# marja-w/gan-des-midi-music-gen

Measured on AMD Instinct MI355X. Metric: GAN training samples/sec (G+D step), higher is better.
Workload: dtype bf16; 1 GPU; SIMNN G/D iteration, synthetic 128x256 spectrogram windows; per_gpu_batch=256, global_batch=256, mode=faithful, parallelism=dp1

## Files before the change

gan_des_midi_music_gen_amd/_lib.py:

```python
import ctypes
import os
import threading

_PKG = os.path.dirname(os.path.abspath(__file__))
_TAG = os.environ.get("GDM_LIB_TAG", "")
LIB_PATH = os.path.join(_PKG, "libgdm_hip" + (f"_{_TAG}" if _TAG else "") + ".so")

F32, BF16 = 0, 1
ACT_NONE, ACT_RELU, ACT_LEAKY, ACT_SIGMOID = 0, 1, 2, 3

_c = ctypes
_P, _I, _L, _F, _Z = _c.c_void_p, _c.c_int, _c.c_int64, _c.c_float, _c.c_size_t

class LinearBnJob(_c.Structure):
    _fields_ = [(n, _P) for n in ("x", "w", "bias", "gamma", "beta", "running_mean", "running_var",
                                  "num_batches_tracked", "y_out", "out", "save_mean", "save_invstd")] + \
               [(n, _I) for n in ("M", "N", "K", "groups", "stat_repeats")]


class DcnnAdam(_c.Structure):
    _fields_ = [("param", _P * 6), ("exp_avg", _P * 6), ("exp_avg_sq", _P * 6), ("hyper", _P), ("done", _P)]


class ConcatJob(_c.Structure):
    _fields_ = [("a", _P), ("b", _P), ("out", _P), ("M", _I), ("Ka", _I), ("Kb", _I)]


SIGNATURES = {
    "gdm_last_error": (_c.c_char_p, []),
    "gdm_version": (_I, []),
    "gdm_arch": (_c.c_char_p, []),
    "gdm_build_flavor": (_I, []),
    "gdm_gemm": (_I, [_P, _I, _L, _L, _P, _I, _L, _L, _P, _I, _L, _L, _I, _I, _I, _P, _P, _I, _F, _I, _I, _P, _Z, _P]),
    "gdm_bce_with_logits": (_I, [_P, _F, _I, _F, _P, _P, _I, _I, _P]),
    "gdm_adam_step": (_I, [_P, _P, _P, _P, _L, _I, _F, _F, _F, _F, _F, _P]),
    "gdm_adam_step_dev": (_I, [_P, _P, _P, _P, _L, _P, _P]),
    "gdm_adam_step_dev_pc": (_I, [_P, _P, _P, _P, _I, _I, _I, _P, _I, _P, _I, _P]),
    "gdm_stft_frames": (_I, [_P, _I, _L, _L, _I, _I, _I, _P, _P]),
    "gdm_power_spectrum": (_I, [_P, _L, _I, _I, _P, _P]),
    "gdm_power_to_db": (_I, [_P, _I, _I, _I, _F, _F, _P, _P]),
    "gdm_bn_workspace_bytes": (_Z, [_I, _I]),
    "gdm_bn_act_fwd": (_I, [_P, _I, _I, _P, _P, _P, _P, _P, _F, _F, _I, _P, _I, _P, _P, _I, _P, _Z, _P]),
    "gdm_bn_act_bwd": (_I, [_P, _P, _I, _P, _I, _I, _P, _P, _P, _I, _P, _P, _P, _P, _Z, _P]),
    "gdm_bn_stats": (_I, [_P, _I, _I, _P, _P, _P, _F, _F, _P, _P, _P, _Z, _P]),
    "gdm_bn_partial_chunks": (_I, [_I]),
    "gdm_bn_partials": (_I, [_P, _I, _I, _P, _P]),
    "gdm_bn_apply": (_I, [_P, _I, _I, _P, _P, _P, _P, _I, _P, _I, _P]),
    "gdm_bn_finalize": (_I, [_P, _I, _I, _I, _F, _F, _P, _P, _P, _P, _P, _P]),
    "gdm_simnn_gen_pack_bytes": (_Z, []),
    "gdm_simnn_gen_pack": (_I, [_P, _I, _P, _P, _P, _P]),
    "gdm_simnn_gen_first": (_I, [_P, _I, _I, _P, _P, _F, _F, _P, _P, _P, _P, _P, _P]),
    "gdm_simnn_gen_convt_chunks": (_I, [_I, _I]),
    "gdm_simnn_gen_convt_bn": (_I, [_I, _P, _P, _P, _P, _P, _I, _P, _P, _P, _P]),
    "gdm_simnn_gen_last": (_I, [_P, _P, _P, _P, _P, _P, _I, _P, _P]),
    "gdm_bias_act_fwd": (_I, [_P, _P, _I, _I, _I, _F, _P, _I, _P]),
    "gdm_act_bwd": (_I, [_P, _P, _I, _L, _I, _F, _P, _P]),
    "gdm_colsum": (_I, [_P, _I, _I, _I, _P, _P, _Z, _P]),
    "gdm_cast": (_I, [_P, _I, _P, _I, _L, _P]),
    "gdm_nonfinite_count": (_I, [_P, _I, _L, _P, _P]),
    "gdm_simnn_conv1_fwd": (_I, [_P, _P, _P, _I, _I, _I, _P, _P, _I, _P]),
    "gdm_simnn_conv1_fwd_pair": (_I, [_P, _P, _I, _P, _P, _I, _I, _I, _P, _P, _I, _P]),
    "gdm_simnn_conv2_pack_bytes": (_Z, [_I]),
    "gdm_simnn_conv2_pack": (_I, [_P, _I, _P, _P]),
    "gdm_simnn_conv2_fwd": (_I, [_P, _P, _P, _I, _I, _I, _P, _P, _I, _P]),
    "gdm_simnn_conv2_bwd_fused_workspace_bytes": (_Z, [_I, _I, _I]),
    "gdm_simnn_conv2_bwd_fused": (_I, [_P, _P, _P, _I, _I, _I, _P, _P, _P, _I, _I, _I, _P, _I, _P, _Z, _P]),
    "gdm_simnn_conv2_bwd_fused_finish": (_I, [_I, _I, _I, _P, _P, _P, _Z, _P]),
    "gdm_simnn_conv2_bwd_data": (_I, [_P, _P, _P, _I, _I, _I, _P, _I, _P]),
    "gdm_simnn_conv2_bwd_weight_workspace_bytes": (_Z, [_I, _I, _I]),
    "gdm_simnn_conv2_bwd_weight": (_I, [_P, _P, _P, _I, _I, _I, _P, _P, _I, _P, _Z, _P]),
    "gdm_simnn_conv1_bwd_weight_workspace_bytes": (_Z, [_I, _I, _I]),
    "gdm_simnn_conv1_bwd_weight": (_I, [_P, _P, _P, _I, _I, _I, _P, _P, _I, _I, _P, _Z, _P]),
    "gdm_simnn_conv1_bwd_data": (_I, [_P, _P, _P, _I, _I, _I, _P, _I, _P]),
    "gdm_simnn_adam_step": (_I, [_P, _P, _P, _P, _I, _I, _I, _P, _P, _P, _P, _P, _I, _P, _P, _I, _P, _P, _P]),
    "gdm_simnn_head_workspace_bytes": (_Z, [_I]),
    "gdm_simnn_head": (_I, [_P, _P, _P, _I, _I, _F, _F, _P, _P, _I, _P, _I, _P, _P, _P, _P, _Z, _P]),
    "gdm_linear_bn_act_max_rows": (_I, []),
    "gdm_linear_bn_act_fwd_multi": (_I, [_P, _I, _F, _F, _I, _I, _P]),
    "gdm_concat_cols_multi": (_I, [_P, _I, _P]),
    "gdm_linear_bn_act_fwd": (_I, [_P, _P, _P, _P, _P, _P, _P, _P, _F, _F, _I, _I, _I, _I, _I, _P, _P, _P, _P, _I, _I,
                                   _P]),
    "gdm_dcnn_fused_supported": (_I, [_I]),
    "gdm_dcnn_pack_bytes": (_Z, [_I]),
    "gdm_dcnn_pack": (_I, [_P, _P, _P, _P, _P, _P, _I, _P, _P]),
    "gdm_dcnn_fused_workspace_bytes": (_Z, [_I, _I, _I]),
    "gdm_dcnn_fused": (_I, [_P, _I, _P, _P, _I, _I, _F, _F, _P, _P, _P, _I, _I, _P, _P, _P, _P, _P, _P, _P, _Z, _P]),
# ... 44 lines not shown
```

gan_des_midi_music_gen_amd/functional.py:

```python
import contextlib

import torch

from . import ops
from .ops import ACT_LEAKY, ACT_NONE, ACT_RELU, ACT_SIGMOID, BF16, F32

_DEFAULT = {"dtype": F32}
_NAMES = {"fp32": F32, "f32": F32, "float32": F32, "bf16": BF16, "bfloat16": BF16, F32: F32, BF16: BF16}


def set_compute_dtype(name):
    _DEFAULT["dtype"] = _NAMES[name]


def get_compute_dtype():
    return _DEFAULT["dtype"]


@contextlib.contextmanager
def compute_dtype(name):
    old = _DEFAULT["dtype"]
    _DEFAULT["dtype"] = _NAMES[name]
    try:
        yield
    finally:
        _DEFAULT["dtype"] = old


def _f32c(t):
    return t.detach().contiguous() if t.dtype == torch.float32 else t.detach().float().contiguous()


def simnn_disc_prepare(w2, wf1, dt, out=None):
    n, k = wf1.shape
    if out is not None:
        pack, wf1p = out
        ops.simnn_conv2_pack(w2, dt, out=pack)
        ops.permute_pc(wf1, n, 32, k // 32, out=wf1p)
        return pack, wf1p
    pack = ops.simnn_conv2_pack(w2, dt)
    wf1p = ops.permute_pc(wf1, n, 32, k // 32, out_dtype=dt).view(n, k)
    return pack, wf1p


def simnn_disc_features(x, w1, b1, pack, b2, wf1p, bf1, dt, trunk_out=None):
    if trunk_out is None:
        x = _f32c(x)
        p1, code1 = ops.simnn_conv1_fwd(x, w1, b1, dt)
    else:
        p1, code1 = trunk_out
    p2, code2 = ops.simnn_conv2_fwd(p1, pack, b2)
    b = p1.shape[0]
    flat = p2.view(b, -1)
    if flat.shape[1] != wf1p.shape[1]:
        raise ValueError(f"Discriminator.fc1 expects {wf1p.shape[1]} features but this input gives {flat.shape[1]} "
                         "(construct Discriminator(input_hw=...) for this geometry)")
    h1 = ops.gemm(flat, wf1p.t(), bias_n=bf1, act=ACT_RELU, compute=dt)
    return h1, (x, p1, code1, flat, code2, h1)


def simnn_disc_forward(x, w1, b1, pack, b2, wf1p, bf1, wf2, bf2, dt, trunk_out=None):
    h1, saved = simnn_disc_features(x, w1, b1, pack, b2, wf1p, bf1, dt, trunk_out)
    p = ops.gemm(h1, wf2.t(), bias_n=bf2, act=ACT_SIGMOID, compute=dt)
    return p, saved + (p,)


def simnn_disc_backward_from_dh1(saved, dh1, pack, wf1p, dt, out=None, x_pair=None, w1_for_dx=None):
    x, p1, code1, flat, code2 = saved[:5]
    b = p1.shape[0]
    o = out if out is not None else [None] * 8
    n, k = wf1p.shape
    dwf1p = ops.gemm(dh1.t(), flat, compute=dt)
    dwf1 = ops.permute_pc(dwf1p, n, k // 32, 32, out=o[4]).view(n, k)
    dflat = ops.gemm(dh1, wf1p, compute=dt, out_dtype=dt)
    h1s, w1s = p1.shape[1], p1.shape[2]
    dp2 = dflat.view(b, h1s // 2, w1s // 2, 32)
    dw2, db2 = ops.simnn_conv2_bwd_weight(dp2, code2, p1, out=None if out is None else (o[2], o[3]))
    x0, x1 = x_pair if x_pair is not None else (x, None)
    dw1, db1, dp1 = ops.simnn_conv2_bwd_fused(dp2, code2, pack, code1, x0, x1,
                                              out=None if out is None else (o[0], o[1]), want_dp1=w1_for_dx is not None)
    dx = None
    if w1_for_dx is not None:
        dx = ops.simnn_conv1_bwd_data(dp1, code1, w1_for_dx.contiguous(), x0.shape[1], x0.shape[2])
    return dw1, db1, dw2, db2, dwf1, dx


def simnn_disc_backward(saved, dz, pack, wf1p, wf2, dt, out=None, x_pair=None, w1_for_dx=None):
    h1 = saved[5]
    b = h1.shape[0]
    o = out if out is not None else [None] * 8
    dz = dz.reshape(b, 1).contiguous()
    dwf2 = ops.gemm(dz.t(), h1, compute=dt, out=o[6])
    dbf2 = ops.colsum(dz, out=o[7])
    dh1 = ops.act_bwd(ops.gemm(dz, wf2, compute=dt), h1, act=ACT_RELU)
    dbf1 = ops.colsum(dh1, out=o[5])
    dw1, db1, dw2, db2, dwf1, dx = simnn_disc_backward_from_dh1(saved, dh1, pack, wf1p, dt, out, x_pair, w1_for_dx)
    return dw1, db1, dw2, db2, dwf1, dbf1, dwf2, dbf2, dx


def _anomaly_guard(cls):
    fwd, bwd = cls.forward, cls.backward

    def _tensors(xs):
        out = []
        for x in xs:
            if isinstance(x, torch.Tensor) and x.is_floating_point() and x.is_cuda:
                out.append(x.detach())
            elif isinstance(x, (tuple, list)):
                out.extend(_tensors(x))
        return out

    def forward(ctx, *args):
        if not torch.is_anomaly_enabled():
            return fwd(ctx, *args)
        ops.assert_finite(_tensors(args), f"Function '{cls.__name__}' received")
        out = fwd(ctx, *args)
        ops.assert_finite(_tensors(out if isinstance(out, (tuple, list)) else (out,)), f"Function '{cls.__name__}' returned")
        return out

    def backward(ctx, *grads):
        out = bwd(ctx, *grads)
        if torch.is_anomaly_enabled():
            ops.assert_finite(_tensors(grads), f"Function '{cls.__name__}Backward' received")
            ops.assert_finite(_tensors(out if isinstance(out, (tuple, list)) else (out,)),
                              f"Function '{cls.__name__}Backward' returned nan values:")
        return out

# ... 430 lines not shown
```

gan_des_midi_music_gen_amd/ops.py:

```python
import contextlib
import ctypes
import threading

import torch

from . import _lib
from ._lib import ACT_LEAKY, ACT_NONE, ACT_RELU, ACT_SIGMOID, BF16, F32, GdmError, check

_TORCH_DT = {F32: torch.float32, BF16: torch.bfloat16}


def torch_dtype(dt):
    return _TORCH_DT[dt]


def gdm_dtype(t):
    if t.dtype == torch.float32:
        return F32
    if t.dtype == torch.bfloat16:
        return BF16
    raise GdmError(f"unsupported tensor dtype {t.dtype} (fp32 or bf16 only)")


def _need_gpu(*ts):
# ... 49 lines not shown
def workspace_namespace(ns):
    prev = getattr(_ws_ns, "ns", None)
    _ws_ns.ns = ns
    try:
        yield
    finally:
        _ws_ns.ns = prev


def workspace(nbytes, device):
    key = (device.index, torch.cuda.current_stream(device).cuda_stream, getattr(_ws_ns, "ns", None))
    capturing = torch.cuda.is_current_stream_capturing()
    buf = _ws_cache.get(key)
    if buf is None or buf.numel() < nbytes:
        if buf is not None and (capturing or key in _ws_pinned):
            _ws_retired.append(buf)
        buf = torch.empty(max(int(nbytes), 1 << 20), dtype=torch.uint8, device=device)
        _ws_cache[key] = buf
    if capturing:
        _ws_pinned.add(key)
    return buf


def default_split_k(m, n, k, compute):
    tile, kt = (128, 32) if compute == BF16 else (64, 32)
    tiles = ((m + tile - 1) // tile) * ((n + tile - 1) // tile)
    ktiles = (k + kt - 1) // kt
    if tiles >= 128 or ktiles < 32:
        return 1
    target = 256 if compute == BF16 else 768
    return max(1, min(ktiles // 8, (target + tiles - 1) // tiles))


def gemm(a, b, *, bias_n=None, bias_m=None, act=ACT_NONE, slope=0.0, out_dtype=None, compute=F32, split_k=None,
         out=None):
    _need_gpu(a, b, bias_n, bias_m, out)
    assert a.dim() == 2 and b.dim() == 2 and a.shape[1] == b.shape[0], (a.shape, b.shape)
    m, k = a.shape
    n = b.shape[1]
    if out is None:
        out = torch.empty((m, n), dtype=_TORCH_DT[F32 if out_dtype is None else out_dtype], device=a.device)
    assert out.shape == (m, n)
    if split_k is None:
        split_k = default_split_k(m, n, k, compute)
    ws, ws_bytes = None, 0
    if split_k > 1:
        ws_bytes = split_k * m * n * 4
        ws = workspace(ws_bytes, a.device)
    lib = _lib.load()
    _call("gdm_gemm", _p(a), gdm_dtype(a), a.stride(0), a.stride(1), _p(b), gdm_dtype(b), b.stride(0), b.stride(1),
                       _p(out), gdm_dtype(out), out.stride(0), out.stride(1), m, n, k, _p(bias_n), _p(bias_m), act,
                       float(slope), compute, split_k, _p(ws), ws_bytes, _stream())
    return out


def bce_with_logits(x, target, *, grad_scale=1.0, want_grad=True, fuse_sigmoid_backward=False, loss_out=None,
                    accumulate_loss=False, dx_out=None):
    _need_gpu(x, loss_out, dx_out)
    x = x.reshape(-1)
    assert x.dtype == torch.float32 and x.is_contiguous()
    loss = loss_out if loss_out is not None else torch.empty(1, dtype=torch.float32, device=x.device)
    dx = dx_out if dx_out is not None else (torch.empty_like(x) if want_grad else None)
    if dx is not None:
        assert dx.is_contiguous() and dx.numel() == x.numel() and dx.dtype == torch.float32
    _call("gdm_bce_with_logits", _p(x), float(target), x.numel(), float(grad_scale), _p(loss), _p(dx),
                                           1 if fuse_sigmoid_backward else 0, 1 if accumulate_loss else 0, _stream())
    return loss, dx


def adam_step(p, g, m, v, step, lr, beta1, beta2, eps, grad_scale=1.0):
    _need_gpu(p, g, m, v)
    for t in (p, g, m, v):
        assert t.dtype == torch.float32 and t.is_contiguous() and t.numel() == p.numel()
    _call("gdm_adam_step", _p(p), _p(g), _p(m), _p(v), p.numel(), int(step), float(lr), float(beta1),
                                    float(beta2), float(eps), float(grad_scale), _stream())


def adam_hyper(device, lr, beta1, beta2, eps, grad_scale=1.0, step=0):
    h = torch.zeros(8, dtype=torch.float32)
    h[1], h[2], h[3], h[4], h[5] = lr, beta1, beta2, eps, grad_scale
    h.view(torch.int32)[0] = int(step)
    return h.to(device)


def adam_step_dev(p, g, m, v, hyper):
    _need_gpu(p, g, m, v, hyper)
    assert hyper.numel() == 8 and hyper.dtype == torch.float32
    _call("gdm_adam_step_dev", _p(p), _p(g), _p(m), _p(v), p.numel(), _p(hyper), _stream())


def adam_step_dev_pc(p, g_pc, m, v, n, c, pix, shadow_pc, hyper, advance_step=False):
    _need_gpu(p, g_pc, m, v, shadow_pc, hyper)
    for t in (p, g_pc, m, v):
        assert t.dtype == torch.float32 and t.is_contiguous() and t.numel() == n * c * pix, (t.shape, n, c, pix)
    assert shadow_pc.is_contiguous() and shadow_pc.numel() == n * c * pix
    _call("gdm_adam_step_dev_pc", _p(p), _p(g_pc), _p(m), _p(v), n, c, pix, _p(shadow_pc), gdm_dtype(shadow_pc),
          _p(hyper), 1 if advance_step else 0, _stream())


SIMNN_ADAM_RECORD_INTS = 1056


def simnn_adam_step(p_big, g_big_pc, m_big, v_big, n, c, pix, shadow_pc, p_small, g_small, m_small, v_small, conv2_weight,
                    pack, hyper, done):
    _need_gpu(p_big, g_big_pc, m_big, v_big, shadow_pc, p_small, g_small, m_small, v_small, conv2_weight, pack, hyper, done)
    for t in (p_big, g_big_pc, m_big, v_big):
# ... 609 lines not shown
```

gan_des_midi_music_gen_amd/train.py:

```python
import torch

from . import dp
from . import functional as Fn
from . import ops


class FlatBuffers:

    ALIGN = 64

    def __init__(self, params, extra=0, local=0):
        params = [p for p in params]
        assert params, "no parameters"
        dev = params[0].device
        self.params = params
        self.numel = sum(p.numel() for p in params)
        big = max(range(len(params)), key=lambda i: params[i].numel())
        order = [i for i in range(len(params)) if i != big] + [big]
        n_small = self.numel - params[big].numel()
        assert extra % 4 == 0 and 0 <= local <= extra
        self.n_small = (n_small + self.ALIGN - 1) // self.ALIGN * self.ALIGN
        self.n_pad = self.n_small - n_small
        self.n_extra = extra
        self.n_local = local
# ... 177 lines not shown
            torch.cuda.current_stream().wait_event(self._gen_event)
        return self._last_generated

    def invalidate_weights(self):
        self._prepared = None

    def _refresh_operands(self):
        if self._prepared is not None:
            Fn.simnn_disc_prepare(self.d.views[2], self.d.views[4], self.dt, out=self._prepared)

    def _adam(self):
        wf1 = self.d.views[4]
        n, k = wf1.shape
        d = self.d
        if not self.one_launch_optimizer:
            d.adam(self.lr, self.betas, self.eps, grad_scale=1.0 / self.world, big_pc=(n, 32, k // 32, self._prepared[1]))
            ops.simnn_conv2_pack(d.views[2], self.dt, out=self._prepared[0])
            return
        if getattr(self, "_adam_done", None) is None:
            self._adam_done = d.derived_record = torch.zeros(ops.SIMNN_ADAM_RECORD_INTS, dtype=torch.int32,
                                                             device=d.flat.device)
        want = d.sync_hyper(self.lr, self.betas, self.eps, 1.0 / self.world)
        if d._hyper is None:
            d._hyper = ops.adam_hyper(d.flat.device, *want, step=d.step_count)
            d._hyper_host = want
        d.step_count += 1
        ns = d.n_small
        ops.simnn_adam_step(d.flat[ns:], d.grad[ns:], d.exp_avg[ns:], d.exp_avg_sq[ns:], n, 32, k // 32, self._prepared[1],
                            d.flat[:ns], d.grad[:ns], d.exp_avg[:ns], d.exp_avg_sq[:ns], d.views[2], self._prepared[0],
                            d._hyper, self._adam_done)

    def _gen_state(self):
        g = self.gen
        ws = [g.conv1.weight.detach(), g.conv2.weight.detach(), g.conv3.weight.detach(), g.conv4.weight.detach()]
        bns = [(bn.weight.detach(), bn.bias.detach(), bn.running_mean, bn.running_var, bn.num_batches_tracked)
               for bn in (g.batch_norm1, g.batch_norm2, g.batch_norm3)]
        return ws, bns

    def _streams(self, dev):
        if self._side is None:
            self._side = [torch.cuda.Stream(dev) for _ in range(3)]
        return self._side

    def _d_backward(self, saved, dh, pack, wf1p, outs, x_pair, keep, fork=True):
        dt = self.dt
        x, p1, code1, flat, code2 = saved[:5]
        b = p1.shape[0]
        n, k = wf1p.shape
        main = torch.cuda.current_stream()
        side = self._streams(p1.device) if (self.overlap and fork) else None
        if side:
            side[1].wait_stream(main)
        with torch.cuda.stream(side[1] if side else main):
            ops.gemm(dh.t(), flat, compute=dt, out=outs[4].view(n, k))
            if self.world > 1 and outs is self.d.grad_views:
                self._reduce_big_async()
        dflat = ops.gemm(dh, wf1p, compute=dt, out_dtype=dt)
        h1s, w1s = p1.shape[1], p1.shape[2]
        dp2 = dflat.view(b, h1s // 2, w1s // 2, 32)
        keep.append(dflat)
        ops.simnn_conv2_bwd_weight(dp2, code2, p1, out=(outs[2], outs[3]))
        x0, x1 = x_pair if x_pair is not None else (x, None)
        ops.simnn_conv2_bwd_fused(dp2, code2, pack, code1, x0, x1, out=(outs[0], outs[1]))
        if side:
            main.wait_stream(side[1])

    @torch.no_grad()
    def step(self, real, noise, fake):
        if self._pending_fake is not None:
            self.flush()
        dt = self.dt
        w1, b1, w2, b2, wf1, bf1, wf2, bf2 = self.d.views
        gv = self.d.grad_views
        real = Fn._f32c(real)
        self._watch(real, noise, fake)
        b, h, w = real.shape
        main = torch.cuda.current_stream()
        side = self._streams(real.device) if self.overlap else None
        keep = []
        ws, bns = self._gen_state()

        def generator_forward():
            if side:
                side[0].wait_stream(main)
            with torch.cuda.stream(side[0] if side else main):
                generated, gsaved = Fn.simnn_gen_forward(noise, ws, bns, self.gen.training, dt, cache=self._tm_cache,
                                                           need_backward=False)
                keep.append(gsaved)
            self._last_generated = generated
            return generated

        bridge = callable(fake)
        if bridge:
            generated = generator_forward()
            if side:
                main.wait_stream(side[0])
            fake = fake(generated)
        fake = Fn._f32c(fake.to(real.device))
        assert fake.shape == real.shape, (fake.shape, real.shape)
        if self._prepared is None:
            self._prepared = Fn.simnn_disc_prepare(w2, wf1, dt)
        pack, wf1p = self._prepared
        h1, w1s = (h + 1) // 2, (w + 1) // 2
        adt = ops.torch_dtype(dt)
        p1 = torch.empty((2 * b, h1, w1s, 16), dtype=adt, device=real.device)
        code1 = torch.empty((2 * b, h1, ops.simnn_code1_width(w1s)), dtype=torch.int64, device=real.device)
        ops.simnn_conv1_fwd(real, w1, b1, dt, out=(p1[:b], code1[:b]))
        ops.simnn_conv1_fwd(fake, w1, b1, dt, out=(p1[b:], code1[b:]))
        if not bridge:
            generator_forward()
# ... 131 lines not shown
            with ops.workspace_namespace(("graph", id(self._graph))), torch.cuda.graph(self._graph):
                self.step_pipelined(*self._static, with_generator=False)
        else:
            with ops.workspace_namespace(("graph", id(self._graph))), torch.cuda.graph(self._graph):
                fn(*self._static)
        self.d.step_count -= 1
        self.iterations -= 1
        return self._graph

    def _capture_pieces(self, real, noise, fake):
        real, fake = Fn._f32c(real), Fn._f32c(fake)
        self._static = (real, noise, fake)
        dev = real.device
        warm = torch.cuda.Stream(dev)
        warm.wait_stream(torch.cuda.current_stream())
        with torch.cuda.stream(warm):
            for _ in range(2):
                self.step_pipelined(*self._static)
        torch.cuda.current_stream().wait_stream(warm)
        torch.cuda.synchronize()
        dt = self.dt
        w1, b1, w2, b2, wf1, bf1, wf2, bf2 = self.d.views
        gv = self.d.grad_views
        pack, wf1p = self._prepared
        b, h, w = real.shape
        h1, w1s = (h + 1) // 2, (w + 1) // 2
        adt = ops.torch_dtype(dt)
        g = {k: torch.cuda.CUDAGraph() for k in ("gen", "half", "a", "b", "c")}
        ctx = {}

        def cap(name):
            return ops.workspace_namespace(("graph", id(g[name])))

        with cap("gen"), torch.cuda.graph(g["gen"]):
            ws, bns = self._gen_state()
            self._last_generated, _gs = Fn.simnn_gen_forward(noise, ws, bns, self.gen.training, dt, cache=self._tm_cache,
                                                             need_backward=False)
        with cap("half"), torch.cuda.graph(g["half"]):
            keep = []
            self._generator_half(self._pending_fake, keep)
            self._fake_buf.copy_(fake)
            ctx["half_keep"] = keep
        with cap("a"), torch.cuda.graph(g["a"]):
            p1 = torch.empty((2 * b, h1, w1s, 16), dtype=adt, device=dev)
            code1 = torch.empty((2 * b, h1, ops.simnn_code1_width(w1s)), dtype=torch.int64, device=dev)
            ops.simnn_conv1_fwd(real, w1, b1, dt, out=(p1[:b], code1[:b]))
            ops.simnn_conv1_fwd(fake, w1, b1, dt, out=(p1[b:], code1[b:]))
            hid, saved = Fn.simnn_disc_features(None, w1, b1, pack, b2, wf1p, bf1, dt, trunk_out=(p1, code1))
            _prob, dh, _ = ops.simnn_head(hid, wf2, bf2, b, 0.9, 0.1, loss_out=self.loss_d, grad_out=(gv[6], gv[7], gv[5]),
                                          dh_dtype=dt)
            ctx.update(saved=saved, dh=dh, hid=hid, prob=_prob)
            _x, p1, code1, flat, code2 = saved[:5]
            n, k = wf1p.shape
            ops.gemm(dh.t(), flat, compute=dt, out=gv[4].view(n, k))
        with cap("b"), torch.cuda.graph(g["b"]):
            dflat = ops.gemm(ctx["dh"], wf1p, compute=dt, out_dtype=dt)
            dp2 = dflat.view(2 * b, h1 // 2, w1s // 2, 32)
            ops.simnn_conv2_bwd_weight(dp2, code2, p1, out=(gv[2], gv[3]))
            ops.simnn_conv2_bwd_fused(dp2, code2, pack, code1, real, fake, out=(gv[0], gv[1]))
            ctx["dflat"] = dflat
        with cap("c"), torch.cuda.graph(g["c"]):
            self._adam()
        self.d.step_count -= 1
        self._pieces = (g, ctx)
        self._graph, self._graph_gen = g["a"], None
        self._piece_streams = tuple(torch.cuda.Stream(dev) for _ in range(3))
        return g

    def _replay_pieces(self):
        g, _ctx = self._pieces
        sg, sh, s1 = self._piece_streams
        main = torch.cuda.current_stream()
        sg.wait_stream(main)
        with torch.cuda.stream(sg):
            g["gen"].replay()
            self._gen_event = sg.record_event()
        sh.wait_stream(main)
        with torch.cuda.stream(sh):
            g["half"].replay()
            half_ev = sh.record_event()
        g["a"].replay()
        if self.world > 1:
            s1.wait_stream(main)
            with torch.cuda.stream(s1):
                self._reduce_big_async()
        g["b"].replay()
        self._reduce()
        main.wait_event(half_ev)
        g["c"].replay()
        main.wait_event(self._gen_event)
        self.d.step_count += 1
        self.iterations += 1
        return self.loss_d, self.loss_g

    def replay(self):
        self._sync_hyper()
        if getattr(self, "_pieces", None) is not None:
            return self._replay_pieces()
        main = torch.cuda.current_stream()
        if self._graph_gen is not None:
            sg = self._gen_replay_stream
            sg.wait_stream(main)
            with torch.cuda.stream(sg):
                self._graph_gen.replay()
                self._gen_event = sg.record_event()
        self._graph.replay()
        if self._graph_gen is not None:
            main.wait_event(self._gen_event)
        self.d.step_count += 1
# ... 336 lines not shown
```

include/gdm.h:

```cpp
#ifndef GDM_H
#define GDM_H
#include <stddef.h>
#include <stdint.h>

#ifdef __cplusplus
extern "C" {
#endif

enum { GDM_F32 = 0, GDM_BF16 = 1 };
enum { GDM_ACT_NONE = 0, GDM_ACT_RELU = 1, GDM_ACT_LEAKY = 2, GDM_ACT_SIGMOID = 3 };
enum { GDM_OK = 0, GDM_EINVAL = -1, GDM_ELAUNCH = -2, GDM_EWORKSPACE = -3 };

const char* gdm_last_error(void);
int gdm_version(void);
const char* gdm_arch(void);
int gdm_build_flavor(void);

int gdm_gemm(const void* A, int a_dtype, int64_t sam, int64_t sak,
             const void* B, int b_dtype, int64_t sbk, int64_t sbn,
             void* C, int c_dtype, int64_t scm, int64_t scn,
             int M, int N, int K,
             const float* bias_n, const float* bias_m, int act, float slope,
             int compute_dtype, int split_k, void* workspace, size_t workspace_bytes, void* stream);

int gdm_bce_with_logits(const float* x, float target, int n, float grad_scale, float* loss, float* dx,
                        int fuse_sigmoid_backward, int accumulate_loss, void* stream);

int gdm_adam_step(float* p, const float* g, float* m, float* v, int64_t n, int step, float lr, float beta1,
                  float beta2, float eps, float grad_scale, void* stream);

int gdm_adam_step_dev(float* p, const float* g, float* m, float* v, int64_t n, float* hyper, void* stream);
int gdm_adam_step_dev_pc(float* p, const float* g_pc, float* m, float* v, int N, int C, int P, void* shadow_pc,
                         int shadow_dtype, float* hyper, int advance_step, void* stream);

size_t gdm_bn_workspace_bytes(int rows, int channels);
int gdm_bn_act_fwd(const float* y, int rows, int channels, const float* gamma, const float* beta,
                   float* running_mean, float* running_var, int64_t* num_batches_tracked, float momentum, float eps,
                   int act, void* out, int out_dtype, float* save_mean, float* save_invstd, int training,
                   void* workspace, size_t workspace_bytes, void* stream);
int gdm_bn_act_bwd(const void* dout, const void* out, int out_dtype, const float* y, int rows, int channels,
                   const float* gamma, const float* save_mean, const float* save_invstd, int act, float* dy,
                   float* dgamma, float* dbeta, void* workspace, size_t workspace_bytes, void* stream);
int gdm_bn_stats(const float* y, int rows, int channels, float* running_mean, float* running_var,
                 int64_t* num_batches_tracked, float momentum, float eps, float* save_mean, float* save_invstd,
                 void* workspace, size_t workspace_bytes, void* stream);
int gdm_bn_partial_chunks(int rows);
int gdm_bn_partials(const float* y, int rows, int channels, float* partials, void* stream);
int gdm_bn_apply(const float* y, int rows, int channels, const float* gamma, const float* beta, const float* mean,
                 const float* invstd, int act, void* out, int out_dtype, void* stream);
int gdm_bn_finalize(const float* ws, int chunks, int rows, int channels, float momentum, float eps, float* running_mean,
                    float* running_var, int64_t* num_batches_tracked, float* save_mean, float* save_invstd, void* stream);

size_t gdm_simnn_gen_pack_bytes(void);
int gdm_simnn_gen_pack(const float* w1, int noise_dim, const float* w2, const float* w3, void* pack, void* stream);
int gdm_simnn_gen_first(const float* noise, int B, int noise_dim, const void* pack, float* y1, float momentum, float eps,
                        float* running_mean, float* running_var, int64_t* num_batches_tracked, float* save_mean,
                        float* save_invstd, void* stream);
int gdm_simnn_gen_convt_chunks(int layer, int B);
int gdm_simnn_gen_convt_bn(int layer, const float* yin, const float* mean, const float* invstd, const float* gamma,
                           const float* beta, int B, const void* pack, float* yout, float* ws_partials, void* stream);
int gdm_simnn_gen_last(const float* yin, const float* mean, const float* invstd, const float* gamma, const float* beta,
                       const float* w4, int B, float* out, void* stream);


int gdm_bias_act_fwd(const float* x, const float* bias, int rows, int cols, int act, float slope, void* out,
                     int out_dtype, void* stream);
int gdm_act_bwd(const void* dout, const void* out, int dtype, int64_t n, int act, float slope, void* dx, void* stream);
int gdm_colsum(const void* x, int dtype, int rows, int cols, float* out, void* workspace, size_t workspace_bytes,
               void* stream);
int gdm_cast(const void* src, int src_dtype, void* dst, int dst_dtype, int64_t n, void* stream);
int gdm_nonfinite_count(const void* x, int dtype, int64_t n, int* counter, void* stream);

int gdm_simnn_conv1_fwd(const float* x, const float* w, const float* bias, int B, int H, int W, void* p1,
                        uint64_t* code1, int dtype, void* stream);
int gdm_simnn_conv1_fwd_pair(const float* x0, const float* x1, int bsplit, const float* w, const float* bias, int B,
                             int H, int W, void* p1, uint64_t* code1, int dtype, void* stream);
// ... 115 lines not shown
```

Baseline: 421,800 samples/s.

## Add dedicated fc1 GEMM kernels for discriminator forward, dx and dw

Adds specialised HIP GEMM kernels for the discriminator's fc1 layer with N or K fixed at 128. They use buffer loads, swizzled LDS, transposed LDS reads, register-staged multi-depth prefetch, and a split-K slab plus reduction kernel that applies bias and ReLU for the forward. The forward, dx and dw calls switch from the generic gdm_gemm to these kernels, and the generic path stays as the fallback. The goal is to cut generic-GEMM overhead on these skinny shapes, at the cost of more kernel code and a separate reduction launch in the forward.

```diff
diff --git a/gan_des_midi_music_gen_amd/_lib.py b/gan_des_midi_music_gen_amd/_lib.py
--- a/gan_des_midi_music_gen_amd/_lib.py
+++ b/gan_des_midi_music_gen_amd/_lib.py
@@ -32,6 +32,10 @@
     "gdm_arch": (_c.c_char_p, []),
     "gdm_build_flavor": (_I, []),
     "gdm_gemm": (_I, [_P, _I, _L, _L, _P, _I, _L, _L, _P, _I, _L, _L, _I, _I, _I, _P, _P, _I, _F, _I, _I, _P, _Z, _P]),
+    "gdm_simnn_fc1_fwd_split": (_I, [_I, _I, _I]),
+    "gdm_simnn_fc1_fwd": (_I, [_P, _P, _P, _P, _I, _I, _I, _P, _Z, _P]),
+    "gdm_simnn_fc1_dx": (_I, [_P, _P, _P, _I, _I, _P]),
+    "gdm_simnn_fc1_dw": (_I, [_P, _P, _P, _I, _I, _P]),
     "gdm_bce_with_logits": (_I, [_P, _F, _I, _F, _P, _P, _I, _I, _P]),
     "gdm_adam_step": (_I, [_P, _P, _P, _P, _L, _I, _F, _F, _F, _F, _F, _P]),
     "gdm_adam_step_dev": (_I, [_P, _P, _P, _P, _L, _P, _P]),
diff --git a/gan_des_midi_music_gen_amd/csrc/simnn_fc1.hip b/gan_des_midi_music_gen_amd/csrc/simnn_fc1.hip
--- /dev/null
+++ b/gan_des_midi_music_gen_amd/csrc/simnn_fc1.hip
@@ -0,0 +1,361 @@
+#include "gemm_common.h"
+
+#ifndef GDM_FC1_FWD_DEPTH
+#define GDM_FC1_FWD_DEPTH 4
+#endif
+#ifndef GDM_FC1_DX_DEPTH
+#define GDM_FC1_DX_DEPTH 4
+#endif
+#ifndef GDM_FC1_DW_DEPTH
+#define GDM_FC1_DW_DEPTH 4
+#endif
+
+namespace {
+
+constexpr int BM = 128, BN = 128, NT = 256;
+constexpr int FWD_KT = GDM_GEMM_FAST_KT;
+
+using rsrc_t = __amdgpu_buffer_rsrc_t;
+constexpr uint32_t BUF_OOB = 0x80000000u;
+__device__ __forceinline__ rsrc_t make_rsrc(const void* p, uint32_t bytes) {
+  const uint64_t a = (uint64_t)p;
+  const uint32_t lo = __builtin_amdgcn_readfirstlane((uint32_t)a);
+  const uint32_t hi = __builtin_amdgcn_readfirstlane((uint32_t)(a >> 32));
+  return __builtin_amdgcn_make_buffer_rsrc((void*)(((uint64_t)hi << 32) | lo), 0,
+                                           __builtin_amdgcn_readfirstlane(bytes), 0x00020000);
+}
+
+__device__ __forceinline__ void wave_lds_sync() {
+  __builtin_amdgcn_fence(__ATOMIC_RELEASE, "wavefront");
+  __builtin_amdgcn_wave_barrier();
+  __builtin_amdgcn_fence(__ATOMIC_ACQUIRE, "wavefront");
+}
+
+__device__ __forceinline__ bf16x4 lds_tr16(const __bf16* p) {
+  return __builtin_amdgcn_ds_read_tr16_b64_v4bf16((__attribute__((address_space(3))) bf16x4*)p);
+}
+
+template <int KT> __device__ __forceinline__ int kswz(int row) { return KT == 64 ? ((row >> 1) & 7) : ((row >> 1) & 2); }
+__device__ __forceinline__ int rswz(int k) { return (k & 3) | ((k >> 1) & 4); }
+
+template <int KT> struct Stage {
+  static constexpr int N = 128 * KT * 2 / 16 / NT;
+  f32x4 v[N];
+};
+template <int KT> struct Lane {
+  uint32_t off[Stage<KT>::N];
+  int kl[Stage<KT>::N];
+  int lds[Stage<KT>::N];
+};
+
+template <int KT, bool KMAJ>
+__device__ __forceinline__ void lane_init(Lane<KT>& ln, int64_t ld, int rows, int r0) {
+  const int t = threadIdx.x;
+#pragma unroll
+  for (int i = 0; i < Stage<KT>::N; ++i) {
+    const int c = t + NT * i;
+    int rl, kl;
+    if constexpr (KMAJ) {
+      constexpr int CPR = KT / 8;
+      rl = c / CPR; kl = (c % CPR) * 8;
+      ln.off[i] = (uint32_t)(((int64_t)(r0 + rl) * ld + kl) * 2);
+      ln.lds[i] = rl * KT + 8 * ((kl >> 3) ^ kswz<KT>(rl)) + (kl & 7);
+    } else {
+      kl = c / 16; rl = (c % 16) * 8;
+      ln.off[i] = (uint32_t)(((int64_t)kl * ld + r0 + rl) * 2);
+      ln.lds[i] = kl * 128 + (rl ^ (16 * rswz(kl)));
+    }
+    ln.kl[i] = (r0 + rl < rows) ? kl : -1;
+  }
+}
+
+template <int KT, bool KMAJ>
+__device__ __forceinline__ void stage_load(Stage<KT>& st, const Lane<KT>& ln, rsrc_t rs, int64_t ld, int k0, int kend) {
+  const uint32_t kbytes = (uint32_t)((KMAJ ? (int64_t)k0 : (int64_t)k0 * ld) * 2);
+#pragma unroll
+  for (int i = 0; i < Stage<KT>::N; ++i) {
+    const bool ok = ln.kl[i] >= 0 && k0 + ln.kl[i] < kend;
+    st.v[i] = __builtin_bit_cast(f32x4, __builtin_amdgcn_raw_buffer_load_b128(rs, ok ? kbytes + ln.off[i] : BUF_OOB, 0, 0));
+  }
+}
+
+template <int KT>
+__device__ __forceinline__ void stage_store(const Stage<KT>& st, const Lane<KT>& ln, __bf16* __restrict__ img) {
+#pragma unroll
+  for (int i = 0; i < Stage<KT>::N; ++i) *(f32x4*)(img + ln.lds[i]) = st.v[i];
+}
+
+template <int KT, bool KMAJ>
+__device__ __forceinline__ bf16x8 frag_read(const __bf16* __restrict__ img, int row0, int kk, int lr, int lg) {
+  if constexpr (KMAJ) {
+    const int row = row0 + lr;
+    return *(const bf16x8*)&img[row * KT + 8 * ((4 * kk + lg) ^ kswz<KT>(row))];
+  } else {
+    const int q = lr >> 2, p = lr & 3;
+    const int kr = 32 * kk + 8 * lg + q;
+    const int n = (row0 + 4 * p) ^ (16 * (q | (4 * (lg & 1))));
+    const bf16x4 lo = lds_tr16(&img[kr * 128 + n]);
+    const bf16x4 hi = lds_tr16(&img[(kr + 4) * 128 + n]);
+    return __builtin_shufflevector(lo, hi, 0, 1, 2, 3, 4, 5, 6, 7);
+  }
+}
+
+enum { OUT_SLAB = 0, OUT_BF16 = 1, OUT_F32 = 2 };
+
+struct Fc1Args {
+  const __bf16* A; int64_t lda;
+  const __bf16* B; int64_t ldb;
+  void* C; int64_t ldc;
+  int M, N, K, split;
+};
+
+template <bool A_KMAJ, bool B_KMAJ, int KT, int DEPTH, int OUT>
+__global__ __launch_bounds__(NT) void fc1_gemm(Fc1Args g) {
+  static_assert(DEPTH % 2 == 0, "the two LDS buffers alternate with the register stages");
+  constexpr int IMG = 128 * KT;
+  __shared__ __attribute__((aligned(16))) __bf16 smem[2 * 2 * IMG];
+  const int t = threadIdx.x, l = t & 63, w = t >> 6, wm = w >> 1, wn = w & 1;
+  const int lr = l & 15, lg = l >> 4;
+  const int MT = (g.M + BM - 1) / BM, NTl = (g.N + BN - 1) / BN;
+  const int id = blockIdx.x;
+  const int grp = id / (8 * MT), within = id % (8 * MT);
+  const int outer = grp * 8 + (within & 7), mt = within >> 3;
+  if (outer >= NTl * g.split) return;
+  const int nt = outer % NTl, zs = outer / NTl;
+  const int m0 = mt * BM, n0 = nt * BN;
+  const int kstep = KT * g.split;
+  const int kbeg = zs * KT, kend = g.K;
+  const rsrc_t ra = make_rsrc(g.A, (uint32_t)((A_KMAJ ? (int64_t)(g.M - 1) * g.lda + g.K : (int64_t)(g.K - 1) * g.lda + g.M) * 2));
+  const rsrc_t rb = make_rsrc(g.B, (uint32_t)((B_KMAJ ? (int64_t)(g.N - 1) * g.ldb + g.K : (int64_t)(g.K - 1) * g.ldb + g.N) * 2));
+  Lane<KT> la, lb;
+  lane_init<KT, A_KMAJ>(la, g.lda, g.M, m0);
+  lane_init<KT, B_KMAJ>(lb, g.ldb, g.N, n0);
+
+  f32x4 acc[4][4];
+#pragma unroll
+  for (int i = 0; i < 4; ++i)
+#pragma unroll
+    for (int j = 0; j < 4; ++j) acc[i][j] = (f32x4){0.f, 0.f, 0.f, 0.f};
+
+  Stage<KT> sa[DEPTH], sb[DEPTH];
+#pragma unroll
+  for (int d = 0; d < DEPTH; ++d) {
+    stage_load<KT, A_KMAJ>(sa[d], la, ra, g.lda, kbeg + d * kstep, kend);
+    stage_load<KT, B_KMAJ>(sb[d], lb, rb, g.ldb, kbeg + d * kstep, kend);
+  }
+  for (int k0 = kbeg; k0 < kend; k0 += DEPTH * kstep) {
+#pragma unroll
+    for (int d = 0; d < DEPTH; ++d) {
+      __bf16* As = smem + 2 * IMG * (d & 1);
+      __bf16* Bs = As + IMG;
+      stage_store<KT>(sa[d], la, As);
+      stage_store<KT>(sb[d], lb, Bs);
+      __syncthreads();
+      const int kn = k0 + (d + DEPTH) * kstep;
+      stage_load<KT, A_KMAJ>(sa[d], la, ra, g.lda, kn, kend);
+      stage_load<KT, B_KMAJ>(sb[d], lb, rb, g.ldb, kn, kend);
+#pragma unroll
+      for (int kk = 0; kk < KT / 32; ++kk) {
+        bf16x8 a[4], b[4];
+#pragma unroll
+        for (int i = 0; i < 4; ++i) a[i] = frag_read<KT, A_KMAJ>(As, wm * 64 + 16 * i, kk, lr, lg);
+#pragma unroll
+        for (int j = 0; j < 4; ++j) b[j] = frag_read<KT, B_KMAJ>(Bs, wn * 64 + 16 * j, kk, lr, lg);
+#pragma unroll
+        for (int i = 0; i < 4; ++i)
+#pragma unroll
+          for (int j = 0; j < 4; ++j) acc[i][j] = mfma16(b[j], a[i], acc[i][j]);
+      }
+    }
+  }
+
+  const bool vec_ok = (g.N % 4 == 0);
+  if constexpr (OUT == OUT_SLAB) {
+#pragma unroll
+    for (int i = 0; i < 4; ++i) {
+      const int m = m0 + wm * 64 + 16 * i + lr;
+      if (m >= g.M) continue;
+#pragma unroll
+      for (int j = 0; j < 4; ++j) {
+        const int n = n0 + wn * 64 + 16 * j + 4 * lg;
+        if (n >= g.N) continue;
+        float* dst = (float*)g.C + ((int64_t)zs * g.M + m) * g.N + n;
+        if (vec_ok) __builtin_nontemporal_store(acc[i][j], (f32x4*)dst);
+        else
+          for (int r = 0; r < 4 && n + r < g.N; ++r) dst[r] = acc[i][j][r];
+      }
+    }
+    return;
+  } else {
+    constexpr bool is_bf16 = OUT == OUT_BF16;
+    if (vec_ok && m0 + BM <= g.M && n0 + BN <= g.N && (!is_bf16 || (g.ldc % 8 == 0 && ((uintptr_t)g.C & 15) == 0))) {
+      __syncthreads();
+      float* scr = (float*)smem + w * (16 * 64);
+      const int prow = is_bf16 ? (l >> 3) : (l >> 4), pcol = is_bf16 ? 8 * (l & 7) : 4 * (l & 15);
+      const int nn = n0 + wn * 64 + pcol;
+#pragma unroll
+      for (int i = 0; i < 4; ++i) {
+        wave_lds_sync();
+#pragma unroll
+        for (int j = 0; j < 4; ++j) *(f32x4*)&scr[lr * 64 + 4 * ((4 * j + lg) ^ lr)] = acc[i][j];
+        wave_lds_sync();
+        if constexpr (is_bf16) {
+#pragma unroll
+          for (int h = 0; h < 2; ++h) {
+            const int row = 8 * h + prow, c8 = l & 7;
+            const f32x4 v0 = *(const f32x4*)&scr[row * 64 + 4 * ((2 * c8) ^ row)];
+            const f32x4 v1 = *(const f32x4*)&scr[row * 64 + 4 * ((2 * c8 + 1) ^ row)];
+            const int m = m0 + wm * 64 + 16 * i + row;
+            bf16x8 hv;
+#pragma unroll
+            for (int r = 0; r < 4; ++r) {
+              hv[r] = (__bf16)v0[r];
+              hv[4 + r] = (__bf16)v1[r];
+            }
+            __builtin_nontemporal_store(hv, (bf16x8*)((__bf16*)g.C + (int64_t)m * g.ldc + nn));
+          }
+        } else {
+#pragma unroll
+          for (int h = 0; h < 4; ++h) {
+            const int row = 4 * h + prow, pc = l & 15;
+            const f32x4 v = *(const f32x4*)&scr[row * 64 + 4 * (pc ^ row)];
+            const int m = m0 + wm * 64 + 16 * i + row;
+            __builtin_nontemporal_store(v, (f32x4*)((float*)g.C + (int64_t)m * g.ldc + nn));
+          }
+        }
+      }
+      return;
+    }
+#pragma unroll
+    for (int i = 0; i < 4; ++i) {
+      const int m = m0 + wm * 64 + 16 * i + lr;
+      if (m >= g.M) continue;
+#pragma unroll
+      for (int j = 0; j < 4; ++j) {
+        const int n = n0 + wn * 64 + 16 * j + 4 * lg;
+        if (n >= g.N) continue;
+        for (int r = 0; r < 4 && n + r < g.N; ++r)
+          store_from_f32(g.C, is_bf16 ? GDM_BF16 : GDM_F32, (int64_t)m * g.ldc + n + r, acc[i][j][r]);
+      }
+    }
+  }
+}
+
+template <int Q4>
+__global__ __launch_bounds__(256) void fc1_slab_sum(GemmArgs g) {
+  __shared__ f32x4 part[4][64];
+  const int64_t total = (int64_t)g.M * g.N;
+  const int lane = threadIdx.x & 63, zg = threadIdx.x >> 6;
+  const int64_t idx = ((int64_t)blockIdx.x * 64 + lane) * 4;
+  const bool live = idx < total;
+  const int q4 = (g.split_k + 3) / 4;
+  const int z0 = zg * q4, z1 = min(g.split_k, z0 + q4);
+  const int nz = z1 - z0;
+  f32x4 v[Q4];
+#pragma unroll
+  for (int i = 0; i < Q4; ++i)
+    v[i] = (live && i < nz) ? __builtin_nontemporal_load((const f32x4*)(g.ws + (int64_t)(z0 + i) * total + idx))
+                            : (f32x4){0.f, 0.f, 0.f, 0.f};
+  f32x4 s[4];
+#pragma unroll
+  for (int q = 0; q < 4; ++q) s[q] = (f32x4){0.f, 0.f, 0.f, 0.f};
+  const int n4 = nz > 0 ? nz & ~3 : 0;
+#pragma unroll
+  for (int i = 0; i < Q4; i += 4)
+    if (i < n4) {
+#pragma unroll
+      for (int q = 0; q < 4; ++q) s[q] += v[i + q];
+    }
+#pragma unroll
+  for (int i = 0; i < Q4; ++i)
+    if (i >= n4 && i < nz) s[0] += v[i];
+  part[zg][lane] = (s[0] + s[1]) + (s[2] + s[3]);
+  __syncthreads();
+  if (zg == 0 && live) {
+    const f32x4 r = (part[0][lane] + part[1][lane]) + (part[2][lane] + part[3][lane]);
+    const int m = (int)(idx / g.N), n = (int)(idx % g.N);
+#pragma unroll
+    for (int e = 0; e < 4; ++e) gemm_epilogue_store(g, m, n + e, r[e]);
+  }
+}
+
+int launch_gemm(const Fc1Args& g, bool a_kmaj, bool b_kmaj, int out, hipStream_t s) {
+  const int MT = (g.M + BM - 1) / BM, NTl = (g.N + BN - 1) / BN;
+  const int outer = NTl * g.split;
+  dim3 grid((unsigned)(((outer + 7) / 8) * 8 * MT));
+  if (out == OUT_SLAB && a_kmaj && b_kmaj)
+    hipLaunchKernelGGL((fc1_gemm<true, true, FWD_KT, GDM_FC1_FWD_DEPTH, OUT_SLAB>), grid, dim3(NT), 0, s, g);
+  else if (out == OUT_BF16 && a_kmaj && !b_kmaj)
+    hipLaunchKernelGGL((fc1_gemm<true, false, 32, GDM_FC1_DX_DEPTH, OUT_BF16>), grid, dim3(NT), 0, s, g);
+  else if (out == OUT_F32 && !a_kmaj && !b_kmaj)
+    hipLaunchKernelGGL((fc1_gemm<false, false, 32, GDM_FC1_DW_DEPTH, OUT_F32>), grid, dim3(NT), 0, s, g);
+  else {
+    gdm_set_error("simnn_fc1: no kernel for this layout");
+    return GDM_EINVAL;
+  }
+  GDM_LAUNCH_OK("gdm_simnn_fc1");
+  return GDM_OK;
+}
+
+bool aligned16(const void* p) { return ((uintptr_t)p & 15) == 0; }
+
+}
+
+extern "C" int gdm_simnn_fc1_fwd_split(int M, int K, int split_k) {
+  if (M < 32 || M > 512 || K <= 0 || K % 8 != 0 || split_k < 1) return 0;
+  const int tiles = (K + FWD_KT - 1) / FWD_KT;
+  if (split_k > tiles) split_k = tiles;
+  const int per = (tiles + split_k - 1) / split_k;
+  const int split = (tiles + per - 1) / per;
+  const int MT = (M + BM - 1) / BM;
+  if (split < 2 || split > 256 || split * MT > 512 || per * FWD_KT < 256) return 0;
+  return split;
+}
+
+extern "C" int gdm_simnn_fc1_fwd(const void* p2, const void* w1, const float* bias, float* h1, int M, int K,
+                                 int split_k, void* workspace, size_t workspace_bytes, void* stream) {
+  constexpr int N = 128;
+  GDM_REQUIRE(p2 && w1 && bias && h1, "gdm_simnn_fc1_fwd: null operand");
+  GDM_REQUIRE(M >= 32 && M <= 512 && K > 0 && K % 8 == 0, "gdm_simnn_fc1_fwd: bad shape M=%d K=%d", M, K);
+  GDM_REQUIRE(aligned16(p2) && aligned16(w1) && aligned16(bias) && aligned16(h1), "gdm_simnn_fc1_fwd: unaligned operand");
+  GDM_REQUIRE((int64_t)M * K * 2 < ((int64_t)1 << 31) && (int64_t)N * K * 2 < ((int64_t)1 << 31),
+              "gdm_simnn_fc1_fwd: operand too large");
+  const int split = gdm_simnn_fc1_fwd_split(M, K, split_k);
+  GDM_REQUIRE(split > 0, "gdm_simnn_fc1_fwd: M=%d K=%d split_k=%d is not gdm_gemm's deep split-K path", M, K, split_k);
+  GDM_REQUIRE(workspace && workspace_bytes >= (size_t)split * M * N * sizeof(float),
+              "gdm_simnn_fc1_fwd: split %d needs %zu workspace bytes, got %zu", split,
+              (size_t)split * M * N * sizeof(float), workspace_bytes);
+  hipStream_t s = (hipStream_t)stream;
+  Fc1Args a{(const __bf16*)p2, K, (const __bf16*)w1, K, workspace, N, M, N, K, split};
+  int rc = launch_gemm(a, true, true, OUT_SLAB, s);
+  if (rc != GDM_OK) return rc;
+  GemmArgs g{nullptr, 0, 0, nullptr, 0, 0, h1, GDM_F32, N, 1, M, N, K, bias, nullptr, GDM_ACT_RELU, 0.f,
+             split, 0, (float*)workspace};
+  const dim3 grid((unsigned)(((int64_t)M * N / 4 + 63) / 64));
+  const int q4 = (split + 3) / 4;
+  if (q4 <= 16) hipLaunchKernelGGL(fc1_slab_sum<16>, grid, dim3(256), 0, s, g);
+  else if (q4 <= 32) hipLaunchKernelGGL(fc1_slab_sum<32>, grid, dim3(256), 0, s, g);
+  else hipLaunchKernelGGL(fc1_slab_sum<64>, grid, dim3(256), 0, s, g);
+  GDM_LAUNCH_OK("gdm_simnn_fc1_fwd(slab sum)");
+  return GDM_OK;
+}
+
+extern "C" int gdm_simnn_fc1_dx(const void* dh, const void* w1, void* dp2, int M, int N, void* stream) {
+  constexpr int K = 128;
+  GDM_REQUIRE(dh && w1 && dp2, "gdm_simnn_fc1_dx: null operand");
+  GDM_REQUIRE(M >= 1 && M <= 512 && N > 0 && N % 8 == 0, "gdm_simnn_fc1_dx: bad shape M=%d N=%d", M, N);
+  GDM_REQUIRE(aligned16(dh) && aligned16(w1) && aligned16(dp2), "gdm_simnn_fc1_dx: unaligned operand");
+  GDM_REQUIRE((int64_t)K * N * 2 < ((int64_t)1 << 31), "gdm_simnn_fc1_dx: operand too large");
+  Fc1Args a{(const __bf16*)dh, K, (const __bf16*)w1, N, dp2, N, M, N, K, 1};
+  return launch_gemm(a, true, false, OUT_BF16, (hipStream_t)stream);
+}
+
+extern "C" int gdm_simnn_fc1_dw(const void* dh, const void* p2, float* dw, int M, int N, void* stream) {
+  constexpr int R = 128;
+  GDM_REQUIRE(dh && p2 && dw, "gdm_simnn_fc1_dw: null operand");
+  GDM_REQUIRE(M >= 1 && M <= 512 && N > 0 && N % 8 == 0, "gdm_simnn_fc1_dw: bad shape M=%d N=%d", M, N);
+  GDM_REQUIRE(aligned16(dh) && aligned16(p2) && aligned16(dw), "gdm_simnn_fc1_dw: unaligned operand");
+  GDM_REQUIRE((int64_t)M * N * 2 < ((int64_t)1 << 31), "gdm_simnn_fc1_dw: operand too large");
+  Fc1Args a{(const __bf16*)dh, R, (const __bf16*)p2, N, dw, N, R, N, M, 1};
+  return launch_gemm(a, false, false, OUT_F32, (hipStream_t)stream);
+}
diff --git a/gan_des_midi_music_gen_amd/functional.py b/gan_des_midi_music_gen_amd/functional.py
--- a/gan_des_midi_music_gen_amd/functional.py
+++ b/gan_des_midi_music_gen_amd/functional.py
@@ -55,7 +55,7 @@
     if flat.shape[1] != wf1p.shape[1]:
         raise ValueError(f"Discriminator.fc1 expects {wf1p.shape[1]} features but this input gives {flat.shape[1]} "
                          "(construct Discriminator(input_hw=...) for this geometry)")
-    h1 = ops.gemm(flat, wf1p.t(), bias_n=bf1, act=ACT_RELU, compute=dt)
+    h1 = ops.simnn_fc1_fwd(flat, wf1p, bf1, dt)
     return h1, (x, p1, code1, flat, code2, h1)
 
 
@@ -70,9 +70,9 @@
     b = p1.shape[0]
     o = out if out is not None else [None] * 8
     n, k = wf1p.shape
-    dwf1p = ops.gemm(dh1.t(), flat, compute=dt)
+    dwf1p = ops.simnn_fc1_dw(dh1, flat, dt)
     dwf1 = ops.permute_pc(dwf1p, n, k // 32, 32, out=o[4]).view(n, k)
-    dflat = ops.gemm(dh1, wf1p, compute=dt, out_dtype=dt)
+    dflat = ops.simnn_fc1_dx(dh1, wf1p, dt)
     h1s, w1s = p1.shape[1], p1.shape[2]
     dp2 = dflat.view(b, h1s // 2, w1s // 2, 32)
     dw2, db2 = ops.simnn_conv2_bwd_weight(dp2, code2, p1, out=None if out is None else (o[2], o[3]))
diff --git a/gan_des_midi_music_gen_amd/ops.py b/gan_des_midi_music_gen_amd/ops.py
--- a/gan_des_midi_music_gen_amd/ops.py
+++ b/gan_des_midi_music_gen_amd/ops.py
@@ -125,6 +125,56 @@
                        _p(out), gdm_dtype(out), out.stride(0), out.stride(1), m, n, k, _p(bias_n), _p(bias_m), act,
                        float(slope), compute, split_k, _p(ws), ws_bytes, _stream())
     return out
+
+
+def _fc1_operands_ok(*ts):
+    return all(t.is_cuda and t.dtype == torch.bfloat16 and t.dim() == 2 and t.is_contiguous() and t.data_ptr() % 16 == 0
+               for t in ts)
+
+
+FC1_MAX_ROWS = 512
+
+
+def simnn_fc1_fwd(flat, w1, bias, compute):
+    _need_gpu(flat, w1, bias)
+    m, k = flat.shape
+    if (compute == BF16 and w1.shape == (128, k) and _fc1_operands_ok(flat, w1) and bias.dtype == torch.float32
+            and bias.is_contiguous() and bias.numel() == 128 and bias.data_ptr() % 16 == 0):
+        split = _lib.load().gdm_simnn_fc1_fwd_split(m, k, default_split_k(m, 128, k, compute))
+        if split:
+            out = torch.empty((m, 128), dtype=torch.float32, device=flat.device)
+            ws_bytes = split * m * 128 * 4
+            ws = workspace(ws_bytes, flat.device)
+            _call("gdm_simnn_fc1_fwd", _p(flat), _p(w1), _p(bias), _p(out), m, k, default_split_k(m, 128, k, compute),
+                  _p(ws), ws_bytes, _stream())
+            return out
+    return gemm(flat, w1.t(), bias_n=bias, act=ACT_RELU, compute=compute)
+
+
+def simnn_fc1_dx(dh, w1, compute):
+    _need_gpu(dh, w1)
+    m = dh.shape[0]
+    n = w1.shape[1]
+    if (compute == BF16 and dh.shape == (m, 128) and w1.shape[0] == 128 and 1 <= m <= FC1_MAX_ROWS and n % 8 == 0
+            and _fc1_operands_ok(dh, w1)):
+        out = torch.empty((m, n), dtype=torch.bfloat16, device=dh.device)
+        _call("gdm_simnn_fc1_dx", _p(dh), _p(w1), _p(out), m, n, _stream())
+        return out
+    return gemm(dh, w1, compute=compute, out_dtype=compute)
+
+
+def simnn_fc1_dw(dh, flat, compute, out=None):
+    _need_gpu(dh, flat, out)
+    m, n = flat.shape
+    out_ok = out is None or (out.shape == (128, n) and out.dtype == torch.float32 and out.is_contiguous()
+                             and out.data_ptr() % 16 == 0)
+    if (compute == BF16 and dh.shape == (m, 128) and 1 <= m <= FC1_MAX_ROWS and n % 8 == 0 and out_ok
+            and _fc1_operands_ok(dh, flat)):
+        if out is None:
+            out = torch.empty((128, n), dtype=torch.float32, device=dh.device)
+        _call("gdm_simnn_fc1_dw", _p(dh), _p(flat), _p(out), m, n, _stream())
+        return out
+    return gemm(dh.t(), flat, compute=compute, out=out)
 
 
 def bce_with_logits(x, target, *, grad_scale=1.0, want_grad=True, fuse_sigmoid_backward=False, loss_out=None,
diff --git a/gan_des_midi_music_gen_amd/train.py b/gan_des_midi_music_gen_amd/train.py
--- a/gan_des_midi_music_gen_amd/train.py
+++ b/gan_des_midi_music_gen_amd/train.py
@@ -253,10 +253,10 @@
         if side:
             side[1].wait_stream(main)
         with torch.cuda.stream(side[1] if side else main):
-            ops.gemm(dh.t(), flat, compute=dt, out=outs[4].view(n, k))
+            ops.simnn_fc1_dw(dh, flat, dt, out=outs[4].view(n, k))
             if self.world > 1 and outs is self.d.grad_views:
                 self._reduce_big_async()
-        dflat = ops.gemm(dh, wf1p, compute=dt, out_dtype=dt)
+        dflat = ops.simnn_fc1_dx(dh, wf1p, dt)
         h1s, w1s = p1.shape[1], p1.shape[2]
         dp2 = dflat.view(b, h1s // 2, w1s // 2, 32)
         keep.append(dflat)
@@ -494,9 +494,9 @@
             ctx.update(saved=saved, dh=dh, hid=hid, prob=_prob)
             _x, p1, code1, flat, code2 = saved[:5]
             n, k = wf1p.shape
-            ops.gemm(dh.t(), flat, compute=dt, out=gv[4].view(n, k))
+            ops.simnn_fc1_dw(dh, flat, dt, out=gv[4].view(n, k))
         with cap("b"), torch.cuda.graph(g["b"]):
-            dflat = ops.gemm(ctx["dh"], wf1p, compute=dt, out_dtype=dt)
+            dflat = ops.simnn_fc1_dx(ctx["dh"], wf1p, dt)
             dp2 = dflat.view(2 * b, h1 // 2, w1s // 2, 32)
             ops.simnn_conv2_bwd_weight(dp2, code2, p1, out=(gv[2], gv[3]))
             ops.simnn_conv2_bwd_fused(dp2, code2, pack, code1, real, fake, out=(gv[0], gv[1]))
diff --git a/include/gdm.h b/include/gdm.h
--- a/include/gdm.h
+++ b/include/gdm.h
@@ -22,6 +22,12 @@
              int M, int N, int K,
              const float* bias_n, const float* bias_m, int act, float slope,
              int compute_dtype, int split_k, void* workspace, size_t workspace_bytes, void* stream);
+
+int gdm_simnn_fc1_fwd_split(int M, int K, int split_k);
+int gdm_simnn_fc1_fwd(const void* p2, const void* w1, const float* bias, float* h1, int M, int K, int split_k,
+                      void* workspace, size_t workspace_bytes, void* stream);
+int gdm_simnn_fc1_dx(const void* dh, const void* w1, void* dp2, int M, int N, void* stream);
+int gdm_simnn_fc1_dw(const void* dh, const void* p2, float* dw, int M, int N, void* stream);
 
 int gdm_bce_with_logits(const float* x, float target, int n, float grad_scale, float* loss, float* dx,
                         int fuse_sigmoid_backward, int accumulate_loss, void* stream);
```

New measurement: 426,500 samples/s (median of 6 runs). +1.1%, better.
